# aldma/Bazinga.jl

Hardware: AMD Instinct MI355X
Metric: PANOC inner iterations/sec, n=10^7 l1-quadratic (higher is better)
Workload: dtype f64

## Files before the change

bazinga.jl_amd/csrc/bz_kernels.h:

```cpp
#pragma once
#include <type_traits>

#include <hip/hip_runtime.h>
#include <stdint.h>
#include <math.h>

#include "../../include/bazinga_hip.h"

namespace bz {

constexpr int BLOCK   = 256;
constexpr int WAVES   = BLOCK / 64;
constexpr int PSTRIDE = 2048;

struct ScalarSrc {
    const double* p;
    int count;
    int stride;
};

template <class T> struct PackN;
template <> struct PackN<double> { static constexpr int N = 2; };
template <> struct PackN<float>  { static constexpr int N = 4; };

// ... 208 lines not shown
    constexpr int N = PackN<T>::N;
    if (cnt == N) {
        typename PackVec<T>::type v;
#pragma unroll
        for (int e = 0; e < N; ++e) v[e] = r.v[e];
        __builtin_nontemporal_store(v, reinterpret_cast<typename PackVec<T>::type*>(p + i0));
    } else {
#pragma unroll
        for (int e = 0; e < N; ++e)
            if (e < cnt) p[i0 + e] = r.v[e];
    }
}
template <class T, bool NT>
__device__ __forceinline__ Pack<T> ldo(const T* __restrict__ base, unsigned byte_off) {
    using V = typename PackVec<T>::type;
    const V* p = reinterpret_cast<const V*>(reinterpret_cast<const char*>(base) + byte_off);
    V v;
    if constexpr (NT) v = __builtin_nontemporal_load(p); else v = *p;
    Pack<T> r;
#pragma unroll
    for (int e = 0; e < PackN<T>::N; ++e) r.v[e] = v[e];
    return r;
}
template <class T, bool NT>
__device__ __forceinline__ void sto(T* __restrict__ base, unsigned byte_off, const Pack<T>& r) {
    using V = typename PackVec<T>::type;
    V v;
#pragma unroll
    for (int e = 0; e < PackN<T>::N; ++e) v[e] = r.v[e];
    V* p = reinterpret_cast<V*>(reinterpret_cast<char*>(base) + byte_off);
    if constexpr (NT) __builtin_nontemporal_store(v, p); else *p = v;
}
template <class T> __device__ __forceinline__ Pack<T> splat(T s) {
    Pack<T> r;
#pragma unroll
    for (int e = 0; e < PackN<T>::N; ++e) r.v[e] = s;
    return r;
}

template <class T, class F>
__device__ __forceinline__ void bz_for_chunks(int64_t n, F&& f) {
    constexpr int N = PackN<T>::N;
    const int64_t nfull = n / N;
    const int64_t st = (int64_t)gridDim.x * BLOCK;
    int64_t c = (int64_t)blockIdx.x * BLOCK + threadIdx.x;
    for (; c < nfull; c += st) f(c * N, std::integral_constant<int, N>{});
// ... 2319 lines not shown
            }
        }
        st(s_new, i0, cnt, ps);
        st(y_new, i0, cnt, py);
    });
    block_reduce_store<2>(accF, 0u, parts, slot0 + 5);
    __syncthreads();
    block_reduce_store<NS>(acc, 4u, parts, slot0 + 7);
}

constexpr int FAM_F_ZERO = 0, FAM_F_DIAG = 1;
constexpr int FAM_G_ZERO = 0, FAM_G_L1 = 1, FAM_G_L1NONNEG = 2, FAM_G_L1BOX = 3, FAM_G_INDBOX = 4, FAM_G_INDBOX_VEC = 5;
constexpr int FAM_G_COUNT = 6;
constexpr int FAM_D_ZERO = 0, FAM_D_FREE = 1, FAM_D_BOX = 2, FAM_D_BOX_VEC = 3;
constexpr int FAM_D_VC = 4, FAM_D_CC = 5, FAM_D_EITHEROR = 6, FAM_D_XOR = 7;
constexpr int FAM_D_COUNT = 8;
constexpr int fam_code(int fk, int gk, int dk) { return fk | (gk << 1) | (dk << 4); }
constexpr int fam_fk(int fam) { return fam & 1; }
constexpr int fam_gk(int fam) { return (fam >> 1) & 7; }
constexpr int fam_dk(int fam) { return fam >> 4; }
constexpr int FAM_HEADLINE = fam_code(FAM_F_DIAG, FAM_G_L1, FAM_D_BOX);

template <class T, int MM, bool NT, bool SPEC, bool OFF32 = false, int XR = 0, int UNI = 0, int TRIAL = 0,
          int FAM = FAM_HEADLINE, int PP = 0>
__global__ void __launch_bounds__(BLOCK)
k_fused_compact(CompactVecs<T, MM> V, CompactCoef<MM> C, const T* __restrict__ x,
                const T* __restrict__ res_prev, ElemParams<T> P, T gamma, T* __restrict__ x_d,
                T* __restrict__ z, T* __restrict__ res, T* __restrict__ s_new, T* __restrict__ y_new,
                int64_t n, double* __restrict__ parts, int slot0) {
    constexpr bool FAMILY = XR == 2;
    constexpr int GKC = fam_gk(FAM), DKC = fam_dk(FAM);
    const int fk = FAMILY ? fam_fk(FAM) : (SPEC ? (int)BZ_F_DIAG_QUADRATIC : P.f_kind);
    const int gk = FAMILY ? (GKC >= FAM_G_INDBOX ? (int)BZ_G_IND_BOX : GKC) : (SPEC ? (int)BZ_G_NORM_L1 : P.g_kind);
    const int dk = FAMILY ? (DKC >= FAM_D_VC ? (int)BZ_D_VC_PAIRS + (DKC - FAM_D_VC) : (DKC >= FAM_D_BOX ? (int)BZ_D_BOX : DKC))
                          : (SPEC ? (int)BZ_D_BOX : P.D_kind);
    const int uni = UNI >= 0 ? UNI : C.uni_rt;
    const bool trial = TRIAL >= 0 ? (TRIAL != 0) : (C.trial_rt != 0);
    const int m = SPEC ? MM : V.m;
    T u1[MM], u2h[MM];
    compact_coefs<T, MM>(C, u1, u2h);
    T H0 = (T)C.H0;
    T gl = gamma * P.g_lambda;
    __shared__ unsigned long long gate_sh;
    auto gate_wait = [&]() -> bool {
        if constexpr (XR == 2) {
        if (C.gate_seq != 0ull) {
            static_assert(MM <= 5, "GateRec holds five coefficients of each kind");
// ... 49 lines not shown
    const bool gate_late = PIPE_ && !C.gate_other_stream && C.gate_late;
    if (!gate_late) { if (!gate_wait()) return; }
    if (SPEC && !OFF32) {
#pragma unroll
        for (int i = 0; i < MM; ++i) { asm volatile("" : "+v"(u1[i])); asm volatile("" : "+v"(u2h[i])); }
        asm volatile("" : "+v"(H0));
        asm volatile("" : "+v"(gl));
        asm volatile("" : "+v"(gamma));
    }
    constexpr bool UDIV = XR == 2 && sizeof(T) == 8;
    T rmu_u = T(0), rgam = T(0);
    if constexpr (UDIV) { rgam = T(1) / gamma; if (uni >= 1) rmu_u = T(1) / P.mu_uniform; }
    const T gam0 = (T)C.gam0, gl0 = gam0 * P.g_lambda;
    constexpr int NS = 10 + 4 * MM + 2;
    double acc[NS];
#pragma unroll
    for (int k = 0; k < NS; ++k) acc[k] = 0.0;
    constexpr bool PIPE = SPEC && OFF32 && XR == 2;
    constexpr int NSTREAMS = MM + 1 + (fam_fk(FAM) ? 2 : 0) + (UNI >= 2 ? 0 : (UNI == 1 ? 1 : 2)) + (TRIAL == 0 ? 0 : 1) +
                             (GKC == FAM_G_L1BOX ? 1 : 0) + (GKC == FAM_G_INDBOX_VEC ? 2 : 0) + (DKC == FAM_D_BOX_VEC ? 2 : 0);
    constexpr int DEPTH = NSTREAMS <= 11 ? 2 : 1;
    constexpr bool NTP = NT && PP == 0;
    struct Stage { Pack<T> q, b, mu, muy, px, ps[MM], xt, gu, glo, ghi, dlo, dhi; };
    auto load_stage = [&](Stage& S, unsigned bo) {
        asm volatile("" : "+v"(bo));
        if (fk == BZ_F_DIAG_QUADRATIC) { S.q = ldo<T, NTP>(P.q, bo); S.b = ldo<T, NTP>(P.b, bo); }
        if (uni < 1) S.mu = ldo<T, NT>(P.mu, bo);
        if (uni < 2) S.muy = ldo<T, NT>(P.muy, bo);
        S.px = ldo<T, NT>(x, bo);
        if (trial) S.xt = ldo<T, NT>((const T*)x_d, bo);
#pragma unroll
        for (int i = 0; i < MM; ++i) S.ps[i] = ldo<T, NT>(V.S[i], bo);
        if constexpr (GKC == FAM_G_L1BOX) S.gu = ldo<T, NT>(P.g_u, bo);
        if constexpr (GKC == FAM_G_INDBOX_VEC) {
            S.glo = P.g_lo_vec ? ldo<T, NT>(P.g_lo_vec, bo) : splat(P.g_lo);
            S.ghi = P.g_hi_vec ? ldo<T, NT>(P.g_hi_vec, bo) : splat(P.g_hi);
        }
        if constexpr (DKC == FAM_D_BOX_VEC) {
            S.dlo = P.D_lo_vec ? ldo<T, NT>(P.D_lo_vec, bo) : splat(P.D_lo);
            S.dhi = P.D_hi_vec ? ldo<T, NT>(P.D_hi_vec, bo) : splat(P.D_hi);
        }
    };
    auto body = [&](const int64_t i0, const auto cnt_, const auto staged_, const Stage& SG) {
        const int cnt = cnt_;
        constexpr bool O32 = SPEC && OFF32 && !std::is_integral<std::remove_cv_t<decltype(cnt_)>>::value;
        constexpr bool STAGED = std::remove_cv_t<decltype(staged_)>::value;
        constexpr int N = PackN<T>::N;
        unsigned bo = (unsigned)(i0 * (int64_t)sizeof(T));
        if constexpr (O32) asm volatile("" : "+v"(bo));
        ElemLoads<T> L;
        Pack<T> px, prp, ps[MM], py[MM], d, rmu, pxt;
        if (trial) {
            if constexpr (STAGED) pxt = SG.xt; else pxt = ldp<T, NT>((const T*)x_d, i0, cnt);
        }
        if constexpr (STAGED) {
// ... 133 lines not shown
            if (!trial) sto<T, NT>(x_d, bo, pxd);
            if (z) sto<T, NT>(z, bo, pz);
            if (XR != 2 || res) sto<T, NT>(res, bo, pr);
            if constexpr (XR == 0) { sto<T, NT>(s_new, bo, pss); sto<T, NT>(y_new, bo, pyy); }
        } else {
            if (!trial) stp<T, NT>(x_d, i0, cnt, pxd);
            if (z) stp<T, NT>(z, i0, cnt, pz);
            if (XR != 2 || res) stp<T, NT>(res, i0, cnt, pr);
            if constexpr (XR == 0) {
                stp<T, NT>(s_new, i0, cnt, pss);
                stp<T, NT>(y_new, i0, cnt, pyy);
            }
        }
    };
    if constexpr (PIPE) {
        constexpr int N = PackN<T>::N;
        const int64_t nfull = n / N;
        const int64_t stride = (int64_t)gridDim.x * BLOCK;
        int64_t c = (int64_t)blockIdx.x * BLOCK + threadIdx.x;
        auto clampc = [&](int64_t k) { return k < nfull ? k : (nfull - 1); };
        auto fetch = [&](Stage& S, int64_t k) { load_stage(S, (unsigned)(clampc(k) * N * (int64_t)sizeof(T))); };
        auto use = [&](const Stage& S, int64_t k) { body(k * N, std::integral_constant<int, N>{}, std::true_type{}, S); };
        Stage sa, sb;
        if constexpr (DEPTH == 2) {
            Stage sc;
            if (c < nfull) { fetch(sa, c); fetch(sb, c + stride); }
            if (gate_late) { if (!gate_wait()) return; }
            for (;;) {
                if (c >= nfull) break;
                fetch(sc, c + 2 * stride); use(sa, c); c += stride;
                if (c >= nfull) break;
                fetch(sa, c + 2 * stride); use(sb, c); c += stride;
                if (c >= nfull) break;
                fetch(sb, c + 2 * stride); use(sc, c); c += stride;
            }
        } else {
            if (c < nfull) fetch(sa, c);
            if (gate_late) { if (!gate_wait()) return; }
            for (;;) {
                if (c >= nfull) break;
                fetch(sb, c + stride); use(sa, c); c += stride;
                if (c >= nfull) break;
                fetch(sa, c + stride); use(sb, c); c += stride;
            }
        }
        if (c == nfull && nfull * N < n) body(c * N, (int)(n - nfull * N), std::false_type{}, sa);
    } else {
// ... 654 lines not shown
```

bazinga.jl_amd/csrc/bz_solver.hip:

```cpp
#include "bz_solver.h"

#include <hip/hip_ext.h>

#include <algorithm>
#include <array>
#include <atomic>
#include <chrono>
#include <cmath>
#include <cstdio>
#include <cstdlib>
#include <cstring>
#include <limits>
#include <optional>
#include <type_traits>

namespace bz {

Ctx::~Ctx() {
    for (int r = 0; r < P2P_MAXRANKS; ++r)
        if (mbox_opened[r] && mbox_peer[r]) (void)hipIpcCloseMemHandle(mbox_peer[r]);
    if (mbox_local) (void)hipFree(mbox_local);
    if (comm) (void)ncclCommDestroy(comm);
    if (stream) (void)hipStreamDestroy(stream);
}
// ... 705 lines not shown
    std::vector<DBuf<T>> S_, Y_;
    DBuf<double> parts_, alphas_, send_, recv_;
    double* host_out_ = nullptr;
    double* host_out_dev_ = nullptr;
    unsigned long long collect_seq = 0;
    int grp_first[SL_COUNT], grp_cnt[SL_COUNT];
    int slot_n[SL_COUNT];

    bz_panoc_opts opt{};
    bool active = false, fused_ok = false, gx_valid = false, gz_valid = false;
    bool z_valid = true;
    int xr_run_ = 0;
    int xr_env_ = 2, skipz_env_ = 1;
    int gfc_env_ = 0, trialfuse_env_ = 1, fused_begin_env_ = 1;
    int slackfast_env_ = 1;
    int suc_grid_env_ = 1;
    int stencil_regx_env_ = 1;
    int affblend_env_ = 1;
    int densesmall_env_ = 1;
    int slackkind_env_ = 1;
    int slackdepth_env_ = 1;
    int nt_env_ = -1;
    int keepp_env_ = -1;
    int famrt_env_ = 0;
    bool sy_stale_ = false;
    bool rh_stale_ = false;
    double gring_[NXR] = {0};
    bool res_valid = true;
    void materialize_pairs() {
        if (!sy_stale_) return;
        SnapVecs<T, CM> V;
        std::memset(&V, 0, sizeof(V));
        const int m = (int)order.size();
        for (int i = 0; i <= CM; ++i) {
            const int back = std::max(0, m - i);
            V.XH[i] = X_[(xc - back + NXR) % NXR].p;
            V.RH[i] = RES_[(rc - back + NRR) % NRR].p;
            V.gam[i] = back ? gring_[(xc - back + NXR) % NXR] : (double)gamma;
        }
        for (int i = 0; i < m; ++i) { V.S[i] = S_[order[m - 1 - i]].p; V.Y[i] = Y_[order[m - 1 - i]].p; }
        if (rh_stale_ && slack) {
            mv(2 * ((m + 1) + 2 * m + 2) + pstreams(true, true, true) + (P.uni >= 2 ? 0 : 1), nx);
            launch(C_MISC, k_pairs_from_iterates_slack<T, CM>, grid_y, V, m, P, (const T*)ymul_.p, RES_[rc].p, Z_[zc].p, nx);
            res_valid = true; z_valid = true;
        } else if (rh_stale_) {
            mv((m + 1) + pstreams(true, true, true) + 2 * m + 2);
// ... 92 lines not shown
        }
        double z[CM] = {0};
        for (int k = rank - 1; k >= 0; --k) {
            double acc = b[k];
            for (int j = k + 1; j < rank; ++j) acc -= A[k * CM + j] * z[j];
            z[k] = acc / A[k * CM + k];
        }
        for (int i = 0; i < m; ++i) a[i] = 0.0;
        for (int k = 0; k < rank; ++k) a[perm[k]] = z[k];
    }
    bool compact_ok = false;
    int gm = 0;
    double Gsy[CM * CM], Gyy[CM * CM];
    double p_new_ = 0.0, w_new_ = 0.0;
    bool pw_valid = false;
    double hp_[CM] = {0}, hw_[CM] = {0};

    struct GatePlan {
        const T* S[CM];
        const T* x;
        T* xd;
        double gam0, gamma;
        int uni, gfc, fam, m_now;
        bool nt, table, keep_params;
        bool operator==(const GatePlan& o) const {
            for (int i = 0; i < CM; ++i) if (S[i] != o.S[i]) return false;
            return x == o.x && xd == o.xd && gam0 == o.gam0 && gamma == o.gamma && uni == o.uni && gfc == o.gfc &&
                   fam == o.fam && m_now == o.m_now && nt == o.nt && table == o.table && keep_params == o.keep_params;
        }
    };
    static constexpr double KEEP_PARAMS_BYTES = 256e6;
    bool keep_params(bool nt, bool table, int fam) const {
        if (!nt || table || fam != FAM_HEADLINE) return false;
        return keepp_env_ >= 0 ? keepp_env_ != 0 : (double)n * sizeof(T) * 2 <= KEEP_PARAMS_BYTES;
    }
    hipStream_t cur_ = nullptr, gate_stream_ = nullptr, gate_on_ = nullptr;
    GateRec* gate_host_ = nullptr;
    GateRec* gate_host_dev_ = nullptr;
    DBuf<GateRec> gate_dev_;
    unsigned long long gate_seq_ = 0;
    bool gate_pending_ = false, more_coming_ = false;
    int gate_env_ = 1;
    bool gate_broken_ = false;
    int gate_sabotage_ = 0;
    int64_t n_gate_fallbacks_ = 0;
    GatePlan gate_plan_{};
    double gate_bytes_ = 0.0;
    int64_t n_gated_ = 0, n_gate_aborts_ = 0;
    void gate_alloc() {
        if (gate_host_) return;
        BZ_HIP(hipHostMalloc((void**)&gate_host_, sizeof(GateRec), hipHostMallocMapped));
        std::memset(gate_host_, 0, sizeof(GateRec));
        BZ_HIP(hipHostGetDevicePointer((void**)&gate_host_dev_, gate_host_, 0));
        gate_dev_.alloc(1);
        BZ_HIP(hipStreamCreateWithFlags(&gate_stream_, hipStreamNonBlocking));
    }
    void gate_quiesce() {
        gate_abort();
// ... 1 lines not shown
    }
    bool gate_make_plan(int xc_, int m_now, const double* gring, int xr_run, GatePlan& pl) const {
        const int fam = fused_family();
        static const int spec_env = std::getenv("BZ_SPEC") ? std::atoi(std::getenv("BZ_SPEC")) : 1;
        static const int off32_env = std::getenv("BZ_OFF32") ? std::atoi(std::getenv("BZ_OFF32")) : 1;
        const int nt_env = nt_env_;
        const bool small = off32_env && (double)vcap * sizeof(T) < 4.0e9;
        if (!(xr_env_ >= 2 && small && fam >= 0 && xr_run >= m_now)) return false;
        for (int i = 1; i < m_now; ++i)
            if (gring[(xc_ - m_now + i + NXR) % NXR] != (double)gamma) return false;
        std::memset(&pl, 0, sizeof(pl));
        for (int i = 0; i < CM; ++i) {
            const int slot = (xc_ - std::max(0, m_now - i) + NXR) % NXR;
            pl.S[i] = X_[slot].p;
            if (i == 0) pl.gam0 = gring[slot];
        }
        pl.x = X_[xc_].p; pl.xd = X_[(xc_ + 1) % NXR].p;
        pl.gamma = (double)gamma; pl.uni = uni_; pl.fam = fam; pl.m_now = m_now;
        pl.gfc = gfc_env_ > 0 ? std::min(grid, gfc_env_ * std::max(1, num_cus)) : std::min(grid, std::max(1, num_cus));
        const int streams = (m_now + 1) + pstreams(true, true, true) + 1;
        pl.nt = nt_env >= 0 ? nt_env != 0 : (double)n * sizeof(T) * streams > 340e6;
        pl.table = !(spec_env && fam == FAM_HEADLINE) || famrt_env_;
        pl.keep_params = keep_params(pl.nt, pl.table, fam);
        return true;
    }
    void gate_launch(const GatePlan& pl, CompactCoef<CM> C2, T* zarg, bool trial_unused = false) {
        CompactVecs<T, CM> XV;
        XV.m = CM;
        for (int i = 0; i < CM; ++i) { XV.S[i] = pl.S[i]; XV.Y[i] = nullptr; }
        C2.gam0 = pl.gam0;
        const T gam = (T)pl.gamma;
        if (pl.table) {
            C2.uni_rt = pl.uni; C2.trial_rt = 0;
            static const int famct_env = std::getenv("BZ_FAMCT") ? std::atoi(std::getenv("BZ_FAMCT")) : 1;
            FusedFn<T> fn = (famct_env && !famrt_env_) ? family_kernel<T>(pl.fam, pl.nt, pl.uni) : nullptr;
            const bool ct = fn != nullptr;
            if (!fn) fn = family_kernel<T>(pl.fam, pl.nt, -1);
            if (!fn) throw Error(BZ_ERR_STATE, "no one-pass kernel instantiation for this oracle family");
            form_[C_FUSED_IT] = std::string("k_fused_compact<XR=2,UNI=") + (ct ? std::to_string(pl.uni) : std::string("-1")) + ",NT=" +
                                std::to_string(pl.nt ? 1 : 0) + ",TRIAL=" + (ct ? "0" : "-1") + ",FAM=" + std::to_string(pl.fam) + ">";
            launch(C_FUSED_IT, fn, pl.gfc, XV, C2, pl.x, (const T*)nullptr, P, gam, pl.xd, zarg, (T*)nullptr, (T*)nullptr,
                   (T*)nullptr, n, parts_.p, (int)SL_TRIAL);
        } else {
            form_[C_FUSED_IT] = std::string("k_fused_compact<XR=2,UNI=") + char('0' + pl.uni) + (pl.nt ? ",NT=1" : ",NT=0") + ",TRIAL=0" +
                                (pl.keep_params ? ",PP=1>" : ">");
#define BZ_LAUNCH_G(NT_, UNI_, PP_)                                                                               \
    launch(C_FUSED_IT, k_fused_compact<T, CM, NT_, true, true, 2, UNI_, 0, FAM_HEADLINE, PP_>, pl.gfc, XV, C2, pl.x, \
           (const T*)nullptr, P, gam, pl.xd, zarg, (T*)nullptr, (T*)nullptr, (T*)nullptr, n, parts_.p, (int)SL_TRIAL)
            if (pl.nt && pl.keep_params) { if (pl.uni == 2) BZ_LAUNCH_G(true, 2, 1); else if (pl.uni == 1) BZ_LAUNCH_G(true, 1, 1); else BZ_LAUNCH_G(true, 0, 1); }
            else if (pl.nt) { if (pl.uni == 2) BZ_LAUNCH_G(true, 2, 0); else if (pl.uni == 1) BZ_LAUNCH_G(true, 1, 0); else BZ_LAUNCH_G(true, 0, 0); }
            else { if (pl.uni == 2) BZ_LAUNCH_G(false, 2, 0); else if (pl.uni == 1) BZ_LAUNCH_G(false, 1, 0); else BZ_LAUNCH_G(false, 0, 0); }
#undef BZ_LAUNCH_G
        }
    }
    void gate_prelaunch(const GatePlan& pl) {
        gate_alloc();
        CompactCoef<CM> C2;
        std::memset(&C2, 0, sizeof(C2));
        static const int glate_env = std::getenv("BZ_GATELATE") ? std::atoi(std::getenv("BZ_GATELATE")) : 1;
        C2.gate_late = glate_env;
        static const unsigned spin_env = std::getenv("BZ_GATE_SPIN") ? (unsigned)std::atoll(std::getenv("BZ_GATE_SPIN")) : 0u;
        C2.gate_spin_host = spin_env ? spin_env : GATE_SPIN_HOST;
        C2.gate_spin_dev = spin_env ? 8u * spin_env : GATE_SPIN_DEV;
        C2.gate_seq = ++gate_seq_; C2.gate_host = gate_host_dev_; C2.gate_dev = gate_dev_.p; C2.gate_timeout = ptimeout_dev_;
        const int streams = (pl.m_now + 1) + pstreams(true, true, true) + 1;
        mv(streams);
        gate_bytes_ = pending_bytes_;
        hipStream_t here = cur_;
        gate_on_ = gate_env_ != 2 ? cur_ : ((cur_ == ctx->stream) ? gate_stream_ : ctx->stream);
        C2.gate_other_stream = gate_on_ != cur_ ? 1 : 0;
        cur_ = gate_on_;
        try {
// ... 1053 lines not shown
            persist_sabotage_ = std::getenv("BZ_TEST_PERSIST_TIMEOUT") && std::atoi(std::getenv("BZ_TEST_PERSIST_TIMEOUT")) != 0;
            if (ctx->nranks > 1 && o.persist && M >= 1) {
                launch_b(C_MISC, k_fill_slot, 1, 64, parts_.p, (int)SL_AUX, persist_ok ? 0.0 : 1.0);
                slot_n[SL_AUX] = 1;
                gather(SL_AUX, 1, 1u);
                if (collect({SL_AUX}, 1u)[0] > 0.0) persist_ok = false;
            }
            if (!compact_ok && o.lbfgs_compact == 2 && M >= 1 && M <= CM && dir_kind_ == BZ_DIR_LBFGS && !ctx->multi() && !persist_ok &&
                !generic_)
                compact_ok = true;
        }
        t_begin = std::chrono::steady_clock::now();
        k_ = 1; n_grad = n_prox = n_bt = n_halv = n_fused = n_skips = 0;
        last_nbt = 0; last_fused = false; tau = T(0); last_ys = T(0); fbe_last = T(0);
        xc = 0; rc = 0; zc = 0; z_valid = true; xr_run_ = 0; sy_stale_ = false; rh_stale_ = false; res_valid = true;
        xr_env_ = std::getenv("BZ_XR") ? std::atoi(std::getenv("BZ_XR")) : 2;
        gfc_env_ = std::getenv("BZ_GFC") ? std::atoi(std::getenv("BZ_GFC")) : 0;
        trialfuse_env_ = std::getenv("BZ_TRIALFUSE") ? std::atoi(std::getenv("BZ_TRIALFUSE")) : 1;
        fused_begin_env_ = std::getenv("BZ_FUSED_BEGIN") ? std::atoi(std::getenv("BZ_FUSED_BEGIN")) : 1;
        skipz_env_ = std::getenv("BZ_SKIPZ") ? std::atoi(std::getenv("BZ_SKIPZ")) : 1;
        famrt_env_ = std::getenv("BZ_FAMRT") ? std::atoi(std::getenv("BZ_FAMRT")) : 0;
        nt_env_ = std::getenv("BZ_NT") ? std::atoi(std::getenv("BZ_NT")) : -1;
        keepp_env_ = std::getenv("BZ_KEEPP") ? std::atoi(std::getenv("BZ_KEEPP")) : -1;
        slackfast_env_ = std::getenv("BZ_SLACKFAST") ? std::atoi(std::getenv("BZ_SLACKFAST")) : 1;
        slackkind_env_ = std::getenv("BZ_SLACKKIND") ? std::atoi(std::getenv("BZ_SLACKKIND")) : 1;
        densesmall_env_ = std::getenv("BZ_DENSESMALL") ? std::atoi(std::getenv("BZ_DENSESMALL")) : 1;
        affblend_env_ = std::getenv("BZ_AFFINE_BLEND") ? std::atoi(std::getenv("BZ_AFFINE_BLEND")) : 1;
        stencil_regx_env_ = std::getenv("BZ_STENCIL_REGX") ? std::atoi(std::getenv("BZ_STENCIL_REGX")) : 1;
        suc_grid_env_ = std::getenv("BZ_SUC_GRID") ? std::atoi(std::getenv("BZ_SUC_GRID")) : 1;
        slackdepth_env_ = std::getenv("BZ_SLACKDEPTH") ? std::atoi(std::getenv("BZ_SLACKDEPTH")) : 1;
        gate_env_ = std::getenv("BZ_GATE") ? std::atoi(std::getenv("BZ_GATE")) : (ctx->nranks > 1 ? 0 : 1);
        if (ctx->shared_device || gate_broken_) gate_env_ = 0;
        gate_sabotage_ = std::getenv("BZ_TEST_GATE_TIMEOUT") ? std::atoi(std::getenv("BZ_TEST_GATE_TIMEOUT")) : 0;
        if (gate_env_ && fused_ok) gate_alloc();
        gate_quiesce();
        if (x0_dev != X_[0].p)
            BZ_HIP(hipMemcpyAsync(X_[0].p, x0_dev, n * sizeof(T), hipMemcpyDeviceToDevice, ctx->stream));
        const T eps = std::numeric_limits<T>::epsilon();
        T* x = X_[xc].p;
        const int lip_env = fused_begin_env_;
        if (lip_env && desc.c_kind == BZ_C_IDENTITY && !slack && !dense_f &&
            (desc.f_kind == BZ_F_ZERO || desc.f_kind == BZ_F_DIAG_QUADRATIC)) {
            slot_n[SL_FXD] = slot_n[SL_FXD + 1] = grid;
            mv(2 + pstreams(true, true, false));
            launch(C_ALGRAD, k_begin_lip<T>, grid, (const T*)x, P, GX_.p, n, parts_.p, (int)SL_FXD, (int)SL_AUX);
            gather(SL_FXD, 2, 0u);
// ... 217 lines not shown
        const bool use_compact = compact_ok && (!order.empty() || (fused_ok && fused_family() >= 0) ||
                                                stencil_fast_now || aff_track_);
        const bool use_persist = persist_ok && !order.empty() && !use_compact;
        CompactVecs<T, CM> CV;
        CompactCoef<CM> CC;
        TailArgs<T> tail;
        if (use_compact) { CV = compact_vecs(); CC = compact_prepare(CV); std::memset(&tail, 0, sizeof(tail)); }
        else if (dir_kind_ == BZ_DIR_BROYDEN) { if (!res_valid) ensure_z(); tail = broyden_dir(); }
        else tail = use_persist ? two_loop_persist() : two_loop();
        double gsy[CM] = {0}, gyy[CM] = {0};
        double tp[CM] = {0}, tw[CM] = {0}, tpn = 0.0, twn = 0.0;
        constexpr int NFC = 10 + 4 * CM + 2;
        static_assert(SL_TRIAL + NFC <= SL_AUX, "k_fused_compact's slots overlap the next group");
        const int m_at_trial = (int)order.size();
        bool tail_used = false, z_skipped = false, res_skipped = false;
        unsigned long long tail_ticket = 0;
        bool gram_from_trial = false;
        tau = T(1);
        const int xp = xc, xd = (xc + 1) % NXR, xb = (xc + 2) % NXR;
        const int rp = rc, rn = (rc + 1) % NRR, zp = zc, zn = 1 - zc;
        int xcur = xd;
        bool have_trial = false, fused_this = false, reset_this = false, sep_trial = false;
        bool img_trial = false;
        bool trial_ok = false, trial_nt = false, trial_keep = false;
        bool head_on = false, head_fb = false;
        bool state_imgs = false, halved_here = false;
        int trial_uni = 0, trial_gfc = 0, trial_fam = -1;
        bool trial_table = false;
        CompactVecs<T, CM> trial_XV;
        CompactCoef<CM> trial_CC;
        double sep_p = 0.0, sep_w = 0.0;
        if (fused_ok && use_compact) {
            const int gfc_env = gfc_env_;
            int gfc = std::min(grid, (gfc_env > 0 ? gfc_env : 2) * std::max(1, num_cus));
            const int nt_env = nt_env_;
            static const int spec_env = std::getenv("BZ_SPEC") ? std::atoi(std::getenv("BZ_SPEC")) : 1;
            const int fam = fused_family();
            const bool headline = spec_env && fam == FAM_HEADLINE;
            const bool spec = headline && CV.m == CM;
#define BZ_LAUNCH_FC(NT_, SPEC_)                                                                                  \
    launch(C_FUSED, k_fused_compact<T, CM, NT_, SPEC_>, gfc, CV, CC, (const T*)X_[xp].p, (const T*)RES_[rp].p, P, \
           gamma, X_[xd].p, zstore, RES_[rn].p, S_[spare].p, Y_[spare].p, n, parts_.p, (int)SL_TRIAL)
            const bool near_stop = (double)stop_norm_ <= 10.0 * opt.tol || (k_ <= 20 && opt.tol > 0.0);
            T* const zstore = (skipz_env_ && !near_stop) ? (T*)nullptr : Z_[zn].p;
            z_skipped = zstore == nullptr;
            static const int off32_env = std::getenv("BZ_OFF32") ? std::atoi(std::getenv("BZ_OFF32")) : 1;
            const bool small = off32_env && (double)vcap * sizeof(T) < 4.0e9;
// ... 46 lines not shown
                    else { if (snt) BZ_LAUNCH_SXR_U(true, 0, 0); else BZ_LAUNCH_SXR_U(false, 0, 0); }
                } else if (m_now == CM) { if (snt) BZ_LAUNCH_SXR(true, true, -1, 0, 0); else BZ_LAUNCH_SXR(false, true, -1, 0, 0); }
                else { if (snt) BZ_LAUNCH_SXR(true, false, -1, 0, 0); else BZ_LAUNCH_SXR(false, false, -1, 0, 0); }
#undef BZ_LAUNCH_SXR_U
#undef BZ_LAUNCH_SXR
                sy_stale_ = true; rh_stale_ = true; res_skipped = true;
                trial_ok = false;
            } else if (xr == 2) {
                CompactVecs<T, CM> XV;
                XV.m = CM;
                for (int i = 0; i < CM; ++i) {
                    const int slot = (xc - std::max(0, m_now - i) + NXR) % NXR;
                    XV.S[i] = X_[slot].p;
                    XV.Y[i] = nullptr;
                    if (i == 0) CC.gam0 = gring_[slot];
                }
                const bool table = !headline || famrt_env_;
                GatePlan cur;
                std::memset(&cur, 0, sizeof(cur));
                for (int i = 0; i < CM; ++i) cur.S[i] = XV.S[i];
                cur.x = X_[xp].p; cur.xd = X_[xd].p; cur.gam0 = CC.gam0; cur.gamma = (double)gamma; cur.uni = uni; cur.gfc = gfc;
                cur.fam = fam; cur.m_now = m_now; cur.nt = nt; cur.table = table;
                cur.keep_params = keep_params(nt, table, fam);
                if (gate_pending_ && cur == gate_plan_) {
                    gate_release(CC, zstore);
                } else {
                    gate_abort();
                    mv(xr2_streams + (zstore ? 1 : 0));
                    CompactCoef<CM> C2 = CC;
                    C2.gate_seq = 0ull;
                    gate_launch(cur, C2, zstore);
                }
                sy_stale_ = true; rh_stale_ = true; res_skipped = true;
                const int tf_now = trialfuse_env_;
                trial_ok = tf_now != 0; trial_nt = nt; trial_uni = uni; trial_gfc = gfc; trial_XV = XV; trial_CC = CC;
                trial_table = table; trial_fam = fam; trial_keep = cur.keep_params;
            } else if (xr) {
                CompactVecs<T, CM> XV;
                XV.m = CM;
                for (int i = 0; i < CM; ++i) {
                    XV.S[i] = X_[(xc - CM + i + NXR) % NXR].p;
                    XV.Y[i] = RES_[(rc - CM + i + NRR) % NRR].p;
                }
                mv(2 * (CM + 1) + pstreams(true, true, true) + 2 + (zstore ? 1 : 0));
                form_[C_FUSED] = std::string("k_fused_compact<XR=1") + (nt ? ",NT=1>" : ",NT=0>");
                if (nt)
                    launch(C_FUSED, k_fused_compact<T, CM, true, true, true, 1>, gfc, XV, CC, (const T*)X_[xp].p,
                           (const T*)RES_[rp].p, P, gamma, X_[xd].p, zstore, RES_[rn].p, (T*)nullptr, (T*)nullptr, n, parts_.p,
                           (int)SL_TRIAL);
                else
                    launch(C_FUSED, k_fused_compact<T, CM, false, true, true, 1>, gfc, XV, CC, (const T*)X_[xp].p,
                           (const T*)RES_[rp].p, P, gamma, X_[xd].p, zstore, RES_[rn].p, (T*)nullptr, (T*)nullptr, n, parts_.p,
                           (int)SL_TRIAL);
                sy_stale_ = true;
            } else
#define BZ_LAUNCH_FC3(NT_)                                                                                        \
    launch(C_FUSED, k_fused_compact<T, CM, NT_, true, true>, gfc, CV, CC, (const T*)X_[xp].p, (const T*)RES_[rp].p, P, \
           gamma, X_[xd].p, zstore, RES_[rn].p, S_[spare].p, Y_[spare].p, n, parts_.p, (int)SL_TRIAL)
            if (slack) {
// ... 288 lines not shown
            if (halve) trial_ok = false;
            if (sy_stale_ && !trial_ok && (halve || !(FBE_new <= threshold || k >= max_bt))) materialize_pairs();
            if ((!z_valid || !res_valid) && (halve || !(FBE_new <= threshold || k >= max_bt))) ensure_z();
            if (halve) {
                halved_here = true;
                gamma = gamma * T(0.5); ++n_halv;
                if (gamma < min_gamma)
                    std::fprintf(stderr, "Warning: stepsize `gamma` became too small (%g)\n", (double)gamma);
                sigma = sigma * T(2);
                lbfgs_reset();
                fused_this = false; reset_this = true;
                continue;
            }
            if (FBE_new <= threshold || k >= max_bt) break;
            tau = (k >= max_bt - 1) ? T(0) : tau / T(2);
            ++nbt; ++n_bt;
            mv(3);
            launch(C_MISC, k_blend<T>, grid, (const T*)X_[xd].p, (const T*)Z_[zp].p, tau, T(1) - tau,
                   X_[xb].p, n);
            xcur = xb;
            fused_this = false;
            if (trial_ok) {
                for (int kk = 0; kk < NFC; ++kk) slot_n[SL_TRIAL + kk] = trial_gfc;
#define BZ_LAUNCH_FCT(NT_, UNI_, PP_)                                                                             \
    launch(C_FUSED_IT, k_fused_compact<T, CM, NT_, true, true, 2, UNI_, 1, FAM_HEADLINE, PP_>, trial_gfc, trial_XV, trial_CC, \
           (const T*)X_[xp].p, (const T*)nullptr, P, gamma, X_[xb].p, Z_[zn].p, RES_[rn].p, (T*)nullptr,         \
           (T*)nullptr, n, parts_.p, (int)SL_TRIAL)
                mv((m_at_trial + 1) + pstreams(true, true, true) + 1 + 2);
                if (trial_table) {
                    trial_CC.uni_rt = trial_uni; trial_CC.trial_rt = 1;
                    FusedFn<T> fn = family_kernel<T>(trial_fam, trial_nt);
                    form_[C_FUSED_IT] = "k_fused_compact<XR=2,UNI=-1,NT=" + std::to_string(trial_nt ? 1 : 0) + ",TRIAL=-1,FAM=" + std::to_string(trial_fam) + ">";
                    launch(C_FUSED_IT, fn, trial_gfc, trial_XV, trial_CC, (const T*)X_[xp].p, (const T*)nullptr, P, gamma,
                           X_[xb].p, Z_[zn].p, RES_[rn].p, (T*)nullptr, (T*)nullptr, n, parts_.p, (int)SL_TRIAL);
                } else {
                form_[C_FUSED_IT] = std::string("k_fused_compact<XR=2,UNI=") + char('0' + trial_uni) + (trial_nt ? ",NT=1" : ",NT=0") + ",TRIAL=1" +
                                    (trial_keep ? ",PP=1>" : ">");
                if (trial_nt && trial_keep) { if (trial_uni == 2) BZ_LAUNCH_FCT(true, 2, 1); else if (trial_uni == 1) BZ_LAUNCH_FCT(true, 1, 1); else BZ_LAUNCH_FCT(true, 0, 1); }
                else if (trial_nt) { if (trial_uni == 2) BZ_LAUNCH_FCT(true, 2, 0); else if (trial_uni == 1) BZ_LAUNCH_FCT(true, 1, 0); else BZ_LAUNCH_FCT(true, 0, 0); }
                else { if (trial_uni == 2) BZ_LAUNCH_FCT(false, 2, 0); else if (trial_uni == 1) BZ_LAUNCH_FCT(false, 1, 0); else BZ_LAUNCH_FCT(false, 0, 0); }
                }
#undef BZ_LAUNCH_FCT
                if (ctx->p2p_on) {
                    tail_ticket = exchange_collect(SL_TRIAL, NFC, 1u << 9);
                    tail_used = true;
                } else {
                    gather(SL_TRIAL, NFC, 1u << 9);
                    tail_used = false;
                }
                have_trial = true; gram_from_trial = true; gx_valid = false; gz_valid = false;
                n_grad += 2; n_prox += 1;
            } else if (affblend_env_ && aff_track_ && state_imgs && gx_valid && nbt == 1 && !halved_here && compact_ok && !generic_ &&
                       !ctx->multi() && aff_count_ + 1 < aff_refresh_) {
                ++aff_count_; img_trial = true;
                ++n_affine_blends_;
                mv(3, ny);
                launch(C_MISC, k_blend<T>, grid_y, (const T*)CXD_.p, (const T*)CZS_.p, tau, T(1) - tau, CZN_.p, ny);
                std::swap(CXD_.p, CZN_.p); std::swap(CXD_.n, CZN_.n);
                mv(3);
                launch(C_MISC, k_blend<T>, grid, (const T*)GX_.p, (const T*)GZ_.p, tau, T(1) - tau, GZN_.p, n);
                std::swap(GX_.p, GZN_.p); std::swap(GX_.n, GZN_.n);
// ... 104 lines not shown
```

Before: 7174.

## Stream fused-kernel inputs through a per-wave LDS ring via global_load_lds

Adds an LQ variant of the fused compact kernel. It issues global_load_lds_dwordx4 asynchronous copies of all input streams into a multi-slot, per-wave LDS ring, waits on vmcnt, and reads each stage from LDS instead of holding prefetched packs in registers. It is enabled by default for f64 non-temporal headline launches, in both the gated and the trial paths. The aim is deeper memory-level parallelism without register pressure, at the cost of a large LDS footprint per block (which may cut occupancy), inline asm that manipulates M0, and extra LDS read traffic.

```diff
diff --git a/bazinga.jl_amd/csrc/bz_kernels.h b/bazinga.jl_amd/csrc/bz_kernels.h
--- a/bazinga.jl_amd/csrc/bz_kernels.h
+++ b/bazinga.jl_amd/csrc/bz_kernels.h
@@ -1,4 +1,5 @@
 #pragma once
+#include <algorithm>
 #include <type_traits>
 
 #include <hip/hip_runtime.h>
@@ -254,6 +255,36 @@
     for (int e = 0; e < PackN<T>::N; ++e) r.v[e] = v[e];
     return r;
 }
+#define BZ_GLDS_POL_1 " nt"
+#define BZ_GLDS_POL_0 ""
+#define BZ_GLDS_HEAD "s_mov_b32 %0, m0\n\ts_mov_b32 m0, %2\n\ts_nop 0\n\t"
+#define BZ_GLDS_TAIL "s_mov_b32 m0, %0"
+#define BZ_GLDS_L(j, off, P) "global_load_lds_dwordx4 %1, %" #j " offset:" #off P "\n\t"
+#define BZ_GLDS_ASM(P)                                                                                                       \
+    if constexpr (K == 1)                                                                                                    \
+        asm volatile(BZ_GLDS_HEAD BZ_GLDS_L(3, 0, P) BZ_GLDS_TAIL : "=&s"(keep) : "v"(byte_off), "s"(m0v), "s"(b[0]) : "memory"); \
+    else if constexpr (K == 2)                                                                                               \
+        asm volatile(BZ_GLDS_HEAD BZ_GLDS_L(3, 0, P) BZ_GLDS_L(4, 1024, P) BZ_GLDS_TAIL                                     \
+                     : "=&s"(keep) : "v"(byte_off), "s"(m0v), "s"(b[0]), "s"(b[1]) : "memory");                              \
+    else if constexpr (K == 3)                                                                                               \
+        asm volatile(BZ_GLDS_HEAD BZ_GLDS_L(3, 0, P) BZ_GLDS_L(4, 1024, P) BZ_GLDS_L(5, 2048, P) BZ_GLDS_TAIL               \
+                     : "=&s"(keep) : "v"(byte_off), "s"(m0v), "s"(b[0]), "s"(b[1]), "s"(b[2]) : "memory");                   \
+    else                                                                                                                     \
+        asm volatile(BZ_GLDS_HEAD BZ_GLDS_L(3, 0, P) BZ_GLDS_L(4, 1024, P) BZ_GLDS_L(5, 2048, P) BZ_GLDS_L(6, 3072, P)      \
+                     BZ_GLDS_TAIL : "=&s"(keep) : "v"(byte_off), "s"(m0v), "s"(b[0]), "s"(b[1]), "s"(b[2]), "s"(b[3]) : "memory");
+template <bool NT, int K>
+__device__ __forceinline__ void glds16x(const void* const* b, unsigned byte_off, unsigned lds) {
+    static_assert(K >= 1 && K <= 4, "one M0 write covers at most four 1 KiB destinations (13-bit instruction offset)");
+    unsigned keep;
+    const unsigned m0v = __builtin_amdgcn_readfirstlane(lds);
+    if constexpr (NT) { BZ_GLDS_ASM(BZ_GLDS_POL_1) } else { BZ_GLDS_ASM(BZ_GLDS_POL_0) }
+}
+#undef BZ_GLDS_ASM
+#undef BZ_GLDS_L
+#undef BZ_GLDS_TAIL
+#undef BZ_GLDS_HEAD
+#undef BZ_GLDS_POL_0
+#undef BZ_GLDS_POL_1
 template <class T, bool NT>
 __device__ __forceinline__ void sto(T* __restrict__ base, unsigned byte_off, const Pack<T>& r) {
     using V = typename PackVec<T>::type;
@@ -2619,7 +2650,7 @@
 constexpr int FAM_HEADLINE = fam_code(FAM_F_DIAG, FAM_G_L1, FAM_D_BOX);
 
 template <class T, int MM, bool NT, bool SPEC, bool OFF32 = false, int XR = 0, int UNI = 0, int TRIAL = 0,
-          int FAM = FAM_HEADLINE, int PP = 0>
+          int FAM = FAM_HEADLINE, int PP = 0, int LQ = 0>
 __global__ void __launch_bounds__(BLOCK)
 k_fused_compact(CompactVecs<T, MM> V, CompactCoef<MM> C, const T* __restrict__ x,
                 const T* __restrict__ res_prev, ElemParams<T> P, T gamma, T* __restrict__ x_d,
@@ -2715,15 +2746,20 @@
     constexpr int DEPTH = NSTREAMS <= 11 ? 2 : 1;
     constexpr bool NTP = NT && PP == 0;
     struct Stage { Pack<T> q, b, mu, muy, px, ps[MM], xt, gu, glo, ghi, dlo, dhi; };
+    using PolQB = std::integral_constant<bool, NTP>;
+    using PolNT = std::integral_constant<bool, NT>;
+    auto for_fixed_streams = [&](Stage& S, auto&& f) {
+        if (fk == BZ_F_DIAG_QUADRATIC) { f(S.q, P.q, PolQB{}); f(S.b, P.b, PolQB{}); }
+        if (uni < 1) f(S.mu, P.mu, PolNT{});
+        if (uni < 2) f(S.muy, P.muy, PolNT{});
+        f(S.px, x, PolNT{});
+        if (trial) f(S.xt, (const T*)x_d, PolNT{});
+#pragma unroll
+        for (int i = 0; i < MM; ++i) f(S.ps[i], V.S[i], PolNT{});
+    };
     auto load_stage = [&](Stage& S, unsigned bo) {
         asm volatile("" : "+v"(bo));
-        if (fk == BZ_F_DIAG_QUADRATIC) { S.q = ldo<T, NTP>(P.q, bo); S.b = ldo<T, NTP>(P.b, bo); }
-        if (uni < 1) S.mu = ldo<T, NT>(P.mu, bo);
-        if (uni < 2) S.muy = ldo<T, NT>(P.muy, bo);
-        S.px = ldo<T, NT>(x, bo);
-        if (trial) S.xt = ldo<T, NT>((const T*)x_d, bo);
-#pragma unroll
-        for (int i = 0; i < MM; ++i) S.ps[i] = ldo<T, NT>(V.S[i], bo);
+        for_fixed_streams(S, [&](Pack<T>& d, const T* p, auto pol) { d = ldo<T, decltype(pol)::value>(p, bo); });
         if constexpr (GKC == FAM_G_L1BOX) S.gu = ldo<T, NT>(P.g_u, bo);
         if constexpr (GKC == FAM_G_INDBOX_VEC) {
             S.glo = P.g_lo_vec ? ldo<T, NT>(P.g_lo_vec, bo) : splat(P.g_lo);
@@ -2903,7 +2939,77 @@
         auto fetch = [&](Stage& S, int64_t k) { load_stage(S, (unsigned)(clampc(k) * N * (int64_t)sizeof(T))); };
         auto use = [&](const Stage& S, int64_t k) { body(k * N, std::integral_constant<int, N>{}, std::true_type{}, S); };
         Stage sa, sb;
-        if constexpr (DEPTH == 2) {
+        if constexpr (LQ) {
+            static_assert(FAM == FAM_HEADLINE && N * sizeof(T) == 16, "the LDS ring serves the headline family's 16-byte packs");
+            constexpr int SLOTB = NSTREAMS * 64 * 16;
+            constexpr int LQ_R = std::min(4, (160 * 1024 - 2048) / (WAVES * SLOTB));
+            static_assert(LQ_R >= 3 && (LQ_R - 2) * NSTREAMS <= 63, "ring depth / vmcnt range");
+            constexpr int NQB = 2, NNT = NSTREAMS - NQB;
+            __shared__ __attribute__((aligned(16))) unsigned char lq_ring[WAVES * LQ_R * SLOTB];
+            const unsigned wave_off = (threadIdx.x >> 6) * (unsigned)(LQ_R * SLOTB);
+            const unsigned ring_lds = (unsigned)(uintptr_t)lq_ring + wave_off;
+            const unsigned lane_off = (threadIdx.x & 63) * 16u;
+            const void* lq_base[NSTREAMS];
+            {
+                int j = 0;
+                Stage none;
+                for_fixed_streams(none, [&](Pack<T>&, const T* p, auto) {
+                    const int g = j < NQB ? j : (j - NQB) % 4;
+                    lq_base[j++] = (const void*)((uintptr_t)p - 1024u * (unsigned)g);
+                });
+            }
+            auto lq_fetch = [&](unsigned slot, int64_t k) {
+                unsigned bo = (unsigned)(clampc(k) * N * (int64_t)sizeof(T));
+                asm volatile("" : "+v"(bo));
+                asm volatile("s_waitcnt lgkmcnt(0)" ::: "memory");
+                const unsigned dst = ring_lds + slot;
+                static_assert(fam_fk(FAM) == FAM_F_DIAG, "q and b lead the slot");
+                glds16x<NTP, NQB>(lq_base, bo, dst);
+#pragma unroll
+                for (int g = 0; g < NNT; g += 4) {
+                    const unsigned d = dst + 1024u * (unsigned)(NQB + g);
+                    if (NNT - g >= 4) glds16x<NT, 4>(lq_base + NQB + g, bo, d);
+                    else if (NNT - g == 3) glds16x<NT, 3>(lq_base + NQB + g, bo, d);
+                    else if (NNT - g == 2) glds16x<NT, 2>(lq_base + NQB + g, bo, d);
+                    else glds16x<NT, 1>(lq_base + NQB + g, bo, d);
+                }
+            };
+            auto lq_read = [&](Stage& S, unsigned slot) {
+                const unsigned char* src = lq_ring + wave_off + slot + lane_off;
+                for_fixed_streams(S, [&](Pack<T>& d, const T*, auto) {
+                    const typename PackVec<T>::type v = *reinterpret_cast<const typename PackVec<T>::type*>(src);
+#pragma unroll
+                    for (int e = 0; e < N; ++e) d.v[e] = v[e];
+                    src += 1024;
+                });
+            };
+            auto lq_wait = [&]() { asm volatile("s_waitcnt vmcnt(%0)" ::"n"((LQ_R - 2) * NSTREAMS) : "memory"); };
+            auto next_slot = [](unsigned s) { return s + SLOTB == (unsigned)(LQ_R * SLOTB) ? 0u : s + SLOTB; };
+            if (c < nfull) {
+#pragma unroll
+                for (int r = 0; r < LQ_R - 1; ++r) lq_fetch(r * SLOTB, c + r * stride);
+            }
+            if (gate_late) {
+                if (!gate_wait()) { asm volatile("s_waitcnt vmcnt(0)" ::: "memory"); return; }
+            }
+            unsigned sc = 0, sn = (LQ_R - 1) * SLOTB;
+            if (c < nfull) { lq_wait(); lq_read(sa, sc); }
+            auto step = [&](const Stage& cur, Stage& nxt) {
+                lq_fetch(sn, c + (LQ_R - 1) * stride);
+                lq_wait();
+                sc = next_slot(sc); sn = next_slot(sn);
+                lq_read(nxt, sc);
+                use(cur, c);
+                c += stride;
+            };
+            for (;;) {
+                if (c >= nfull) break;
+                step(sa, sb);
+                if (c >= nfull) break;
+                step(sb, sa);
+            }
+            asm volatile("s_waitcnt vmcnt(0)" ::: "memory");
+        } else if constexpr (DEPTH == 2) {
             Stage sc;
             if (c < nfull) { fetch(sa, c); fetch(sb, c + stride); }
             if (gate_late) { if (!gate_wait()) return; }
diff --git a/bazinga.jl_amd/csrc/bz_solver.hip b/bazinga.jl_amd/csrc/bz_solver.hip
--- a/bazinga.jl_amd/csrc/bz_solver.hip
+++ b/bazinga.jl_amd/csrc/bz_solver.hip
@@ -751,6 +751,7 @@
     int slackdepth_env_ = 1;
     int nt_env_ = -1;
     int keepp_env_ = -1;
+    int ldsq_env_ = -1;
     int famrt_env_ = 0;
     bool sy_stale_ = false;
     bool rh_stale_ = false;
@@ -889,11 +890,12 @@
         T* xd;
         double gam0, gamma;
         int uni, gfc, fam, m_now;
-        bool nt, table, keep_params;
+        bool nt, table, keep_params, lds_ring;
         bool operator==(const GatePlan& o) const {
             for (int i = 0; i < CM; ++i) if (S[i] != o.S[i]) return false;
             return x == o.x && xd == o.xd && gam0 == o.gam0 && gamma == o.gamma && uni == o.uni && gfc == o.gfc &&
-                   fam == o.fam && m_now == o.m_now && nt == o.nt && table == o.table && keep_params == o.keep_params;
+                   fam == o.fam && m_now == o.m_now && nt == o.nt && table == o.table && keep_params == o.keep_params &&
+                   lds_ring == o.lds_ring;
         }
     };
     static constexpr double KEEP_PARAMS_BYTES = 256e6;
@@ -901,6 +903,7 @@
         if (!nt || table || fam != FAM_HEADLINE) return false;
         return keepp_env_ >= 0 ? keepp_env_ != 0 : (double)n * sizeof(T) * 2 <= KEEP_PARAMS_BYTES;
     }
+    bool lds_ring(bool nt, bool table) const { return sizeof(T) == 8 && nt && !table && ldsq_env_ != 0; }
     hipStream_t cur_ = nullptr, gate_stream_ = nullptr, gate_on_ = nullptr;
     GateRec* gate_host_ = nullptr;
     GateRec* gate_host_dev_ = nullptr;
@@ -948,6 +951,7 @@
         pl.nt = nt_env >= 0 ? nt_env != 0 : (double)n * sizeof(T) * streams > 340e6;
         pl.table = !(spec_env && fam == FAM_HEADLINE) || famrt_env_;
         pl.keep_params = keep_params(pl.nt, pl.table, fam);
+        pl.lds_ring = lds_ring(pl.nt, pl.table);
         return true;
     }
     void gate_launch(const GatePlan& pl, CompactCoef<CM> C2, T* zarg, bool trial_unused = false) {
@@ -969,11 +973,17 @@
                    (T*)nullptr, n, parts_.p, (int)SL_TRIAL);
         } else {
             form_[C_FUSED_IT] = std::string("k_fused_compact<XR=2,UNI=") + char('0' + pl.uni) + (pl.nt ? ",NT=1" : ",NT=0") + ",TRIAL=0" +
-                                (pl.keep_params ? ",PP=1>" : ">");
-#define BZ_LAUNCH_G(NT_, UNI_, PP_)                                                                               \
-    launch(C_FUSED_IT, k_fused_compact<T, CM, NT_, true, true, 2, UNI_, 0, FAM_HEADLINE, PP_>, pl.gfc, XV, C2, pl.x, \
-           (const T*)nullptr, P, gam, pl.xd, zarg, (T*)nullptr, (T*)nullptr, (T*)nullptr, n, parts_.p, (int)SL_TRIAL)
-            if (pl.nt && pl.keep_params) { if (pl.uni == 2) BZ_LAUNCH_G(true, 2, 1); else if (pl.uni == 1) BZ_LAUNCH_G(true, 1, 1); else BZ_LAUNCH_G(true, 0, 1); }
+                                (pl.keep_params ? ",PP=1" : "") + (pl.lds_ring ? ",LQ=1>" : ">");
+#define BZ_LAUNCH_G(NT_, UNI_, PP_, ...)                                                                          \
+    launch(C_FUSED_IT, k_fused_compact<T, CM, NT_, true, true, 2, UNI_, 0, FAM_HEADLINE, PP_, ##__VA_ARGS__>, pl.gfc, XV, C2, \
+           pl.x, (const T*)nullptr, P, gam, pl.xd, zarg, (T*)nullptr, (T*)nullptr, (T*)nullptr, n, parts_.p, (int)SL_TRIAL)
+            if (pl.lds_ring) {
+                if constexpr (sizeof(T) == 8) {
+                    if (pl.keep_params) { if (pl.uni == 2) BZ_LAUNCH_G(true, 2, 1, 1); else if (pl.uni == 1) BZ_LAUNCH_G(true, 1, 1, 1); else BZ_LAUNCH_G(true, 0, 1, 1); }
+                    else { if (pl.uni == 2) BZ_LAUNCH_G(true, 2, 0, 1); else if (pl.uni == 1) BZ_LAUNCH_G(true, 1, 0, 1); else BZ_LAUNCH_G(true, 0, 0, 1); }
+                }
+            }
+            else if (pl.nt && pl.keep_params) { if (pl.uni == 2) BZ_LAUNCH_G(true, 2, 1); else if (pl.uni == 1) BZ_LAUNCH_G(true, 1, 1); else BZ_LAUNCH_G(true, 0, 1); }
             else if (pl.nt) { if (pl.uni == 2) BZ_LAUNCH_G(true, 2, 0); else if (pl.uni == 1) BZ_LAUNCH_G(true, 1, 0); else BZ_LAUNCH_G(true, 0, 0); }
             else { if (pl.uni == 2) BZ_LAUNCH_G(false, 2, 0); else if (pl.uni == 1) BZ_LAUNCH_G(false, 1, 0); else BZ_LAUNCH_G(false, 0, 0); }
 #undef BZ_LAUNCH_G
@@ -2073,6 +2083,7 @@
         famrt_env_ = std::getenv("BZ_FAMRT") ? std::atoi(std::getenv("BZ_FAMRT")) : 0;
         nt_env_ = std::getenv("BZ_NT") ? std::atoi(std::getenv("BZ_NT")) : -1;
         keepp_env_ = std::getenv("BZ_KEEPP") ? std::atoi(std::getenv("BZ_KEEPP")) : -1;
+        ldsq_env_ = std::getenv("BZ_LDSQ") ? std::atoi(std::getenv("BZ_LDSQ")) : -1;
         slackfast_env_ = std::getenv("BZ_SLACKFAST") ? std::atoi(std::getenv("BZ_SLACKFAST")) : 1;
         slackkind_env_ = std::getenv("BZ_SLACKKIND") ? std::atoi(std::getenv("BZ_SLACKKIND")) : 1;
         densesmall_env_ = std::getenv("BZ_DENSESMALL") ? std::atoi(std::getenv("BZ_DENSESMALL")) : 1;
@@ -2336,7 +2347,7 @@
         int xcur = xd;
         bool have_trial = false, fused_this = false, reset_this = false, sep_trial = false;
         bool img_trial = false;
-        bool trial_ok = false, trial_nt = false, trial_keep = false;
+        bool trial_ok = false, trial_nt = false, trial_keep = false, trial_lq = false;
         bool head_on = false, head_fb = false;
         bool state_imgs = false, halved_here = false;
         int trial_uni = 0, trial_gfc = 0, trial_fam = -1;
@@ -2429,6 +2440,7 @@
                 cur.x = X_[xp].p; cur.xd = X_[xd].p; cur.gam0 = CC.gam0; cur.gamma = (double)gamma; cur.uni = uni; cur.gfc = gfc;
                 cur.fam = fam; cur.m_now = m_now; cur.nt = nt; cur.table = table;
                 cur.keep_params = keep_params(nt, table, fam);
+                cur.lds_ring = lds_ring(nt, table);
                 if (gate_pending_ && cur == gate_plan_) {
                     gate_release(CC, zstore);
                 } else {
@@ -2441,7 +2453,7 @@
                 sy_stale_ = true; rh_stale_ = true; res_skipped = true;
                 const int tf_now = trialfuse_env_;
                 trial_ok = tf_now != 0; trial_nt = nt; trial_uni = uni; trial_gfc = gfc; trial_XV = XV; trial_CC = CC;
-                trial_table = table; trial_fam = fam; trial_keep = cur.keep_params;
+                trial_table = table; trial_fam = fam; trial_keep = cur.keep_params; trial_lq = cur.lds_ring;
             } else if (xr) {
                 CompactVecs<T, CM> XV;
                 XV.m = CM;
@@ -2776,9 +2788,9 @@
             fused_this = false;
             if (trial_ok) {
                 for (int kk = 0; kk < NFC; ++kk) slot_n[SL_TRIAL + kk] = trial_gfc;
-#define BZ_LAUNCH_FCT(NT_, UNI_, PP_)                                                                             \
-    launch(C_FUSED_IT, k_fused_compact<T, CM, NT_, true, true, 2, UNI_, 1, FAM_HEADLINE, PP_>, trial_gfc, trial_XV, trial_CC, \
-           (const T*)X_[xp].p, (const T*)nullptr, P, gamma, X_[xb].p, Z_[zn].p, RES_[rn].p, (T*)nullptr,         \
+#define BZ_LAUNCH_FCT(NT_, UNI_, PP_, ...)                                                                        \
+    launch(C_FUSED_IT, k_fused_compact<T, CM, NT_, true, true, 2, UNI_, 1, FAM_HEADLINE, PP_, ##__VA_ARGS__>, trial_gfc, trial_XV, \
+           trial_CC, (const T*)X_[xp].p, (const T*)nullptr, P, gamma, X_[xb].p, Z_[zn].p, RES_[rn].p, (T*)nullptr,         \
            (T*)nullptr, n, parts_.p, (int)SL_TRIAL)
                 mv((m_at_trial + 1) + pstreams(true, true, true) + 1 + 2);
                 if (trial_table) {
@@ -2789,8 +2801,14 @@
                            X_[xb].p, Z_[zn].p, RES_[rn].p, (T*)nullptr, (T*)nullptr, n, parts_.p, (int)SL_TRIAL);
                 } else {
                 form_[C_FUSED_IT] = std::string("k_fused_compact<XR=2,UNI=") + char('0' + trial_uni) + (trial_nt ? ",NT=1" : ",NT=0") + ",TRIAL=1" +
-                                    (trial_keep ? ",PP=1>" : ">");
-                if (trial_nt && trial_keep) { if (trial_uni == 2) BZ_LAUNCH_FCT(true, 2, 1); else if (trial_uni == 1) BZ_LAUNCH_FCT(true, 1, 1); else BZ_LAUNCH_FCT(true, 0, 1); }
+                                    (trial_keep ? ",PP=1" : "") + (trial_lq ? ",LQ=1>" : ">");
+                if (trial_lq) {
+                    if constexpr (sizeof(T) == 8) {
+                        if (trial_keep) { if (trial_uni == 2) BZ_LAUNCH_FCT(true, 2, 1, 1); else if (trial_uni == 1) BZ_LAUNCH_FCT(true, 1, 1, 1); else BZ_LAUNCH_FCT(true, 0, 1, 1); }
+                        else { if (trial_uni == 2) BZ_LAUNCH_FCT(true, 2, 0, 1); else if (trial_uni == 1) BZ_LAUNCH_FCT(true, 1, 0, 1); else BZ_LAUNCH_FCT(true, 0, 0, 1); }
+                    }
+                }
+                else if (trial_nt && trial_keep) { if (trial_uni == 2) BZ_LAUNCH_FCT(true, 2, 1); else if (trial_uni == 1) BZ_LAUNCH_FCT(true, 1, 1); else BZ_LAUNCH_FCT(true, 0, 1); }
                 else if (trial_nt) { if (trial_uni == 2) BZ_LAUNCH_FCT(true, 2, 0); else if (trial_uni == 1) BZ_LAUNCH_FCT(true, 1, 0); else BZ_LAUNCH_FCT(true, 0, 0); }
                 else { if (trial_uni == 2) BZ_LAUNCH_FCT(false, 2, 0); else if (trial_uni == 1) BZ_LAUNCH_FCT(false, 1, 0); else BZ_LAUNCH_FCT(false, 0, 0); }
                 }
```

New measurement: 7830, median of 6. +9.1%, better.
